# xiaozhah/Aligner

Hardware: AMD Instinct MI355X
Metric: aligned utterances/sec + frames/sec, [B=64,T_text=200,T_mel=1000] (higher is better)
Workload: dtype f32; 1 GPU; configs[1]: similarity (L2, C=80) + monotonic alignment search, [B=64,T_text=200,T_mel=1000] fp32 per GPU, dense fp32 path + int32 durations out; batch_per_gpu=64, t_text=200, t_mel=1000, c_att=80, launch=hipGraph, batches_in_flight=3, parallelism=batch-sharded x1

## Files before the change

aligner_amd/csrc/maxpath.hip:

```cpp
#include <hip/hip_runtime.h>

#include <climits>
#include <cstdint>
#include <cstring>
#include <type_traits>

#include "aligner_amd.h"
#include "common.h"
#include "device.h"
#include "maxpath_sweep_asm.inc"
#include "maxpath_walk_asm.inc"

namespace aligner {

constexpr int TC       = 32;
constexpr int TILE_LD  = 36;
constexpr int RING_T   = 4;
constexpr int RING_LD  = 64;
constexpr int RPW      = 63;
constexpr int WS_HDR_BYTES = 256;
constexpr int MV_CHUNKS = 32;

enum Mode { MODE_NORMAL = 0, MODE_EMPTY = 1, MODE_COMPAT = 2 };

typedef __attribute__((address_space(3))) float lds_float;
typedef float __attribute__((ext_vector_type(4))) f32x4;
typedef __attribute__((address_space(3))) f32x4 lds_f32x4;

struct MaxpathParams {
    const void  *value;
    const void  *mask;
    const int   *t_xs;
    const int   *t_ys;
    int         *starts;
    int         *tok;
    int         *dur;
    unsigned    *bits;
    int         *status;
    int         *mflag;
    int          verify;
    int          redo;
    int          ldv;
    int B, Tx, Ty, NT, ROWS;
    int WT;
    int bits_in_lds;
    int lds_bits_off;
    int lds_prev_off;
    int force_exact;
    float neg;
    int flags;
    float *qout;
    int lds_total;
    unsigned    *xring;
    int         *xflag;
    unsigned    *xwalk;
    int          split_walk;
    unsigned long long *stamps;
    float       *dump;
    void        *path1;
    int          path1_es;
    unsigned long long path1_one;
    int          zero_blocks;
    int          zero_nt;
    unsigned long long zero_n16;
    int         *zsync;
};

#define ALIGNER_STAMP(k)                                                                        \
    do {                                                                                        \
        if (p.stamps && (threadIdx.x & 63) == 0)                                                \
            p.stamps[((size_t)blockIdx.x * 16 + (threadIdx.x >> 6)) * 16 + (k)] =                \
                ((k) == 6 || (k) == 7) ? __builtin_amdgcn_s_memrealtime() : __builtin_amdgcn_s_memtime();   \
    } while (0)

constexpr int ZERO_SPIN_LIMIT = 1 << 22;

enum { VT_F32 = 0, VT_BF16 = 1, VT_F16 = 2 };

template <int VT> __device__ __forceinline__ float half_to_f32(unsigned h16) {
    if (VT == VT_BF16) return __builtin_bit_cast(float, h16 << 16);
    return (float)__builtin_bit_cast(_Float16, (unsigned short)h16);
}
template <int VT> __device__ __forceinline__ float mul_in_dtype(float v, float m) {
    const float r = v * m;
    if (VT == VT_BF16) return (float)(__bf16)r;
    if (VT == VT_F16) return (float)(_Float16)r;
    return r;
}
template <int VT> __device__ __forceinline__ float load_score(const void *base, size_t idx) {
    if (VT == VT_F32) return static_cast<const float *>(base)[idx];
    return half_to_f32<VT>(static_cast<const unsigned short *>(base)[idx]);
}
__device__ __forceinline__ float dpp_wave_shr1(float old_lane0, float src) {
    return __builtin_bit_cast(
        float, __builtin_amdgcn_update_dpp(__builtin_bit_cast(int, old_lane0),
                                           __builtin_bit_cast(int, src),
                                           0x138 , 0xf, 0xf, false));
}

__device__ __forceinline__ float comp(const float4 &v, int i) {
    return i == 0 ? v.x : i == 1 ? v.y : i == 2 ? v.z : v.w;
}

__device__ __forceinline__ int classify_lengths(const MaxpathParams &p, int b, int &tx, int &ty) {
    tx = p.t_xs[b];
    ty = p.t_ys[b];
    int st = 0;
    if (tx > p.Tx) { tx = p.Tx; st |= ALIGNER_ST_CLAMPED; }
    if (ty > p.Ty) { ty = p.Ty; st |= ALIGNER_ST_CLAMPED; }
    int mode;
    if (tx >= 1 && tx <= ty) {
        mode = MODE_NORMAL;
    } else if (ty <= 0) {
        mode = MODE_EMPTY;
        ty = 0;
        if (tx < 0) tx = 0;
    } else if (tx > ty && (p.flags & ALIGNER_F_COMPAT_TXGTTY)) {
        mode = MODE_COMPAT;
    } else {
        mode = MODE_EMPTY;
        st |= ALIGNER_ST_BAD_LENGTHS;
        if (tx < 0) tx = 0;
    }
    if (st && threadIdx.x == 0) atomicOr(p.status, st);
    return mode;
}

__device__ __forceinline__ bool tile_in_band(int t, int r0, int nrows, int tx, int ty) {
    const int y_lo = r0;
    const int y_hi = ty - tx + r0 + nrows - 1;
    return (TC * t + TC - 1 >= y_lo) && (TC * t <= y_hi);
}

__device__ __forceinline__ int starts_words_of(int Tx) { return ((Tx + 1 + 63) / 64) * 64 + 64; }

__device__ __forceinline__ void store_outputs(const MaxpathParams &p, int b, int tx, int ty, int *startsL,
                                              bool distinct_starts = true, int x_lo = 0, int x_hi = -1, int y_lo = 0,
                                              int y_hi = -1) {
    const int tid = threadIdx.x, nthreads = blockDim.x;
    if (p.path1 && p.zero_blocks > 0) {
        int gave_up = 0;
        if (tid == 0) {
            const int limit = (p.flags & ALIGNER_F_TEST_DROP_ZERO_REPORTS) ? (1 << 10) : ZERO_SPIN_LIMIT;
            int spins = 0;
            while (__hip_atomic_load(p.zsync, __ATOMIC_RELAXED, __HIP_MEMORY_SCOPE_AGENT) < p.zero_blocks) {
                if (++spins > limit) { atomicOr(p.status, ALIGNER_ST_INTERNAL); gave_up = 1; break; }
                __builtin_amdgcn_s_sleep(8);
            }
        }
        if (__syncthreads_or(gave_up)) {
            for (int x = tid; x <= p.Tx; x += nthreads) startsL[x] = 0;
            __syncthreads();
            tx = 0;
            ty = 0;
        }
    }
    const int xs_hi = x_hi < 0 ? p.Tx + 1 : x_hi, xd_hi = x_hi < 0 ? p.Tx : x_hi;
    const int ye = y_hi < 0 ? p.Ty : y_hi;
    for (int x = x_lo + tid; x < xs_hi; x += nthreads) p.starts[(size_t)b * (p.Tx + 1) + x] = startsL[x];
    if (p.dur)
        for (int x = x_lo + tid; x < xd_hi; x += nthreads) p.dur[(size_t)b * p.Tx + x] = startsL[x + 1] - startsL[x];
    if (!p.tok && !p.path1) return;
// ... 895 lines not shown
                walk_half(p, win2, RP2, ntb, x, e, 0, startsL + r0, lane);
                e = __builtin_amdgcn_readfirstlane(e);
                if (lane == 0) {
                    unsigned expect = XRING_EMPTY;
                    const bool ok = x == -1 && e >= r0 - 1 &&
                                    __hip_atomic_compare_exchange_strong(p.xwalk + b, &expect, (unsigned)e, __ATOMIC_RELAXED,
                                                                         __ATOMIC_RELAXED, __HIP_MEMORY_SCOPE_AGENT);
                    const bool cancelled = !ok && expect == XWALK_CANCEL;
                    if (!ok && !cancelled) {
                        if (expect == XRING_EMPTY)
                            __hip_atomic_store(p.xwalk + b, XWALK_SOLO, __ATOMIC_RELAXED, __HIP_MEMORY_SCOPE_AGENT);
                        atomicOr(p.status, ALIGNER_ST_INTERNAL);
                    }
                    *bcast = ok ? 1 : cancelled ? 2 : 0;
                }
            }
            ALIGNER_STAMP(3);
            __syncthreads();
            const int handed = *bcast;
            __syncthreads();
            if (handed == 0) {
                write_degenerate<MASKMODE, VT>(p, b, MODE_EMPTY, tx, ty, reinterpret_cast<int *>(smem));
                return;
            }
            if (handed == 1) {
                for (int r = tx + tid; r <= p.Tx; r += NW * 128) startsL[r] = ty;
                __syncthreads();
                store_outputs(p, b, tx, ty, startsL, true, r0, -1, startsL[r0], -1);
                ALIGNER_STAMP(5);
                ALIGNER_STAMP(7);
                return;
            }
            __threadfence_block();
            backtrack_and_store<(NW <= 4)>(p, b, tx, ty, smem);
            return;
        }
        if (p.split_walk && tid == 0) __hip_atomic_store(p.xwalk + b, XWALK_SOLO, __ATOMIC_RELAXED, __HIP_MEMORY_SCOPE_AGENT);
    }
    if (p.force_exact || flagp[0] != 0) exact_fallback_sweep<MASKMODE, VT>(p, b, tx, ty, smem, bitsL, RPB);
    __threadfence_block();
    ALIGNER_STAMP(1);
    backtrack_and_store<(NW <= 4)>(p, b, tx, ty, smem);
    ALIGNER_STAMP(5);
    ALIGNER_STAMP(7);
}

template <int VT, int NTHREADS>
__device__ __forceinline__ void verify_mask_piece(const MaxpathParams &p, int q) {
    constexpr int ES = VT == VT_F32 ? 4 : 2, EPV = 16 / ES, NWV = NTHREADS / 64;
    typedef typename std::conditional<ES == 4, unsigned, unsigned short>::type U;
    const unsigned one_bits = VT == VT_F32 ? 0x3F800000u : VT == VT_BF16 ? 0x3F80u : 0x3C00u;
    const unsigned w1 = ES == 4 ? one_bits : (one_bits | (one_bits << 16));
    const int b = q / MV_CHUNKS, c = q - b * MV_CHUNKS, tid = threadIdx.x, lane = tid & 63, wave = tid >> 6;
    const int tx = p.t_xs[b], ty = p.t_ys[b];
    int bad = 0;
    if (!(tx >= 1 && tx <= ty && tx <= p.Tx && ty <= p.Ty)) {
        bad = 1;
    } else {
        const U *mu = static_cast<const U *>(p.mask) + (size_t)b * p.Tx * p.Ty;
        const int per = (tx + MV_CHUNKS - 1) / MV_CHUNKS;
        const int r0 = c * per, r1 = r0 + per < tx ? r0 + per : tx;
        const bool vec = (p.Ty % EPV == 0) && ((reinterpret_cast<uintptr_t>(p.mask) & 15) == 0);
        const int nq = vec ? ty / EPV : 0;
        for (int x = r0 + wave; x < r1; x += NWV) {
            const uint4 *row = reinterpret_cast<const uint4 *>(mu + (size_t)x * p.Ty);
            int k = lane;
            for (; k + 192 < nq; k += 256) {
                const uint4 v0 = row[k], v1 = row[k + 64], v2 = row[k + 128], v3 = row[k + 192];
                bad |= (v0.x != w1) | (v0.y != w1) | (v0.z != w1) | (v0.w != w1) | (v1.x != w1) | (v1.y != w1) |
                       (v1.z != w1) | (v1.w != w1) | (v2.x != w1) | (v2.y != w1) | (v2.z != w1) | (v2.w != w1) |
                       (v3.x != w1) | (v3.y != w1) | (v3.z != w1) | (v3.w != w1);
            }
            for (; k < nq; k += 64) {
                const uint4 v = row[k];
                bad |= (v.x != w1) | (v.y != w1) | (v.z != w1) | (v.w != w1);
            }
            for (int y = nq * EPV + lane; y < ty; y += 64) bad |= mu[(size_t)x * p.Ty + y] != (U)one_bits;
        }
    }
    const int any = __syncthreads_or(bad);
    if (tid == 0) p.mflag[q] = any;
}

__device__ __forceinline__ void erase_path_ones(const MaxpathParams &p, int b) {
    const int *st = p.starts + (size_t)b * (p.Tx + 1);
    for (int x = threadIdx.x; x < p.Tx; x += blockDim.x) {
        const int s0 = st[x], s1 = st[x + 1];
        for (int y = s0; y < s1 && y < p.Ty; ++y) {
            const size_t idx = ((size_t)b * p.Tx + x) * p.Ty + y;
            switch (p.path1_es) {
                case 1: static_cast<unsigned char *>(p.path1)[idx] = 0; break;
                case 2: static_cast<unsigned short *>(p.path1)[idx] = 0; break;
                case 4: static_cast<unsigned *>(p.path1)[idx] = 0u; break;
                default: static_cast<unsigned long long *>(p.path1)[idx] = 0ull; break;
            }
        }
    }
    asm volatile("s_waitcnt vmcnt(0)" ::: "memory");
    __syncthreads();
}

template <int NW, int DEPTH, bool VEC, int MASKMODE, int VT, bool PAIR = false>
__global__ __launch_bounds__(NW * 128, 1) void maxpath_pipelined_kernel(MaxpathParams p) {
    const int Z = p.zero_blocks;
    if ((int)blockIdx.x < Z) {
        typedef unsigned u32x4 __attribute__((ext_vector_type(4)));
        u32x4 *d = reinterpret_cast<u32x4 *>(p.path1);
        const u32x4 z = {0u, 0u, 0u, 0u};
        const unsigned long long per = (p.zero_n16 + Z - 1) / Z;
        const unsigned long long lo = per * blockIdx.x, hi = lo + per < p.zero_n16 ? lo + per : p.zero_n16;
        if (p.zero_nt) {
            for (unsigned long long i = lo + threadIdx.x; i < hi; i += NW * 128)
                asm volatile("global_store_dwordx4 %0, %1, off sc1 nt" :: "v"(d + i), "v"(z) : "memory");
        } else {
            for (unsigned long long i = lo + threadIdx.x; i < hi; i += NW * 128)
                asm volatile("global_store_dwordx4 %0, %1, off sc1" :: "v"(d + i), "v"(z) : "memory");
        }
        asm volatile("s_waitcnt vmcnt(0)" ::: "memory");
        __syncthreads();
        if (threadIdx.x == 0 && !(p.flags & ALIGNER_F_TEST_DROP_ZERO_REPORTS))
            __hip_atomic_fetch_add(p.zsync, 1, __ATOMIC_RELAXED, __HIP_MEMORY_SCOPE_AGENT);
        if (MASKMODE == 0 && p.verify)
            for (int q = blockIdx.x; q < p.B * MV_CHUNKS; q += Z) verify_mask_piece<VT, NW * 128>(p, q);
    } else if (MASKMODE == 1 && p.redo) {
        const int b = (int)blockIdx.x;
        static_assert(MV_CHUNKS <= 64, "one flag word per lane");
        const int mine = (threadIdx.x & 63) < MV_CHUNKS ? p.mflag[b * MV_CHUNKS + (threadIdx.x & 63)] : 0;
        if (__builtin_amdgcn_ballot_w64(mine != 0) != 0) {
            if (p.path1) erase_path_ones(p, b);
            maxpath_pipelined_body<NW, DEPTH, VEC, 1, VT, PAIR>(p, b);
        }
    } else if (MASKMODE == 2) {
        const int blk = (int)blockIdx.x - Z;
        const int b = PAIR ? (blk >= p.B ? blk - p.B : blk) : blk;
        static_assert(MV_CHUNKS <= 64, "one flag word per lane");
        const int mine = (threadIdx.x & 63) < MV_CHUNKS ? p.mflag[b * MV_CHUNKS + (threadIdx.x & 63)] : 0;
        if (__builtin_amdgcn_ballot_w64(mine != 0) != 0) maxpath_pipelined_body<NW, DEPTH, VEC, 1, VT, PAIR>(p, blk);
        else maxpath_pipelined_body<NW, DEPTH, VEC, 0, VT, PAIR>(p, blk);
    } else {
        maxpath_pipelined_body<NW, DEPTH, VEC, MASKMODE, VT, PAIR>(p, (int)blockIdx.x - Z);
    }
    if (Z > 0) {
        __syncthreads();
        if (threadIdx.x == 0) {
            const int f = __hip_atomic_fetch_add(p.zsync + 1, 1, __ATOMIC_RELAXED, __HIP_MEMORY_SCOPE_AGENT);
            if (f == Z + (PAIR ? 2 : 1) * p.B - 1) {
                __hip_atomic_store(p.zsync, 0, __ATOMIC_RELAXED, __HIP_MEMORY_SCOPE_AGENT);
                __hip_atomic_store(p.zsync + 1, 0, __ATOMIC_RELAXED, __HIP_MEMORY_SCOPE_AGENT);
            }
        }
    }
}

template <typename T, bool VEC, bool STREAM>
__global__ __launch_bounds__(256) void expand_kernel(const int *__restrict__ starts, T *__restrict__ path,
                                                      int Tx, int Ty, int rows_per_block, T one) {
    const int b = blockIdx.z;
    const int x0 = blockIdx.y * rows_per_block;
    const int y0 = (blockIdx.x * 256 + threadIdx.x) * 4;
    if (y0 >= Ty) return;
    const int x1 = (x0 + rows_per_block < Tx) ? x0 + rows_per_block : Tx;
    const int *st = starts + (size_t)b * (Tx + 1);
    struct alignas(sizeof(T) * 4) Vec4 { T v[4]; };
    int s = st[x0];
    for (int x = x0; x < x1; ++x) {
        const int e = st[x + 1];
        T *dst = path + ((size_t)b * Tx + x) * Ty + y0;
        Vec4 o;
#pragma unroll
        for (int i = 0; i < 4; ++i) o.v[i] = (y0 + i >= s && y0 + i < e) ? one : T(0);
        if (VEC) {
            if (STREAM) {
                typedef T TV __attribute__((ext_vector_type(4)));
                TV ov;
                ov.x = o.v[0]; ov.y = o.v[1]; ov.z = o.v[2]; ov.w = o.v[3];
                __builtin_nontemporal_store(ov, reinterpret_cast<TV *>(dst));
            } else {
                *reinterpret_cast<Vec4 *>(dst) = o;
            }
        } else {
#pragma unroll
            for (int i = 0; i < 4; ++i)
                if (y0 + i < Ty) dst[i] = o.v[i];
        }
        s = e;
    }
}

template <typename T, int VT> __device__ __forceinline__ float mask_value(T v) {
    if (VT == VT_F32) return (float)v;
    return half_to_f32<VT>((unsigned)v);
}

template <typename T, int VT = VT_F32>
__global__ __launch_bounds__(256) void lengths_kernel(const T *__restrict__ mask, int Tx, int Ty,
                                                       int *__restrict__ t_xs, int *__restrict__ t_ys) {
    __shared__ float red[2][4];
    const int b = blockIdx.x, tid = threadIdx.x;
    const T *m = mask + (size_t)b * Tx * Ty;
    float sx = 0.f, sy = 0.f;
    for (int x = tid; x < Tx; x += 256) sx += mask_value<T, VT>(m[(size_t)x * Ty]);
    for (int y = tid; y < Ty; y += 256) sy += mask_value<T, VT>(m[y]);
#pragma unroll
    for (int off = 32; off > 0; off >>= 1) {
        sx += __shfl_down(sx, off);
        sy += __shfl_down(sy, off);
    }
    if ((tid & 63) == 0) { red[0][tid >> 6] = sx; red[1][tid >> 6] = sy; }
    __syncthreads();
    if (tid == 0) {
        t_xs[b] = (int)(red[0][0] + red[0][1] + red[0][2] + red[0][3]);
        t_ys[b] = (int)(red[1][0] + red[1][1] + red[1][2] + red[1][3]);
    }
}

template <int ES, int VT>
__global__ __launch_bounds__(256) void mask_verify_kernel(const void *__restrict__ maskv, int Tx, int Ty,
                                                           const int *__restrict__ t_xs_in, const int *__restrict__ t_ys_in,
                                                           int *__restrict__ t_xs_out, int *__restrict__ t_ys_out,
                                                           int *__restrict__ flag, unsigned one_bits) {
    __shared__ float red[2][4];
    __shared__ int anybad;
    typedef typename std::conditional<ES == 4, float, unsigned short>::type E;
    typedef typename std::conditional<ES == 4, unsigned, unsigned short>::type U;
    constexpr int EPV = 16 / ES;
    constexpr int NQ = 4;
    const int c = blockIdx.x, b = blockIdx.y, tid = threadIdx.x, lane = tid & 63, wave = tid >> 6;
    const E *m = static_cast<const E *>(maskv) + (size_t)b * Tx * Ty;
    const U *mu = reinterpret_cast<const U *>(m);
    const U one = (U)one_bits;
    const unsigned w1 = ES == 4 ? one_bits : (one_bits | (one_bits << 16));
    if (tid == 0) anybad = 0;
    const bool given = t_xs_in != nullptr;
    int tx = given ? t_xs_in[b] : -1, ty = given ? t_ys_in[b] : 0;
    const int rows = given ? (tx < Tx ? (tx > 0 ? tx : 0) : Tx) : Tx;
    const int per = (rows + MV_CHUNKS - 1) / MV_CHUNKS;
    const int r0 = c * per, r1 = r0 + per < rows ? r0 + per : rows;
    const bool vec = (Ty % EPV == 0) && ((reinterpret_cast<uintptr_t>(maskv) & 15) == 0);
    const int nqrow = Ty / EPV;
    auto fetch = [&](int x, uint4 (&v)[NQ], U &before) {
        const uint4 *row = reinterpret_cast<const uint4 *>(mu + (size_t)x * Ty);
#pragma unroll
        for (int i = 0; i < NQ; ++i) {
            const int q = lane + 64 * i;
            v[i] = row[q < nqrow ? q : nqrow - 1];
        }
        before = x > 0 ? mu[(size_t)(x - 1) * Ty] : one;
    };
    uint4 v[NQ];
    U before = one;
    int x = r0 + wave;
    if (vec && x < r1) fetch(x, v, before);
    if (!given) {
        float sx = 0.f, sy = 0.f;
        for (int y = tid; y < Ty; y += 256) sy += mask_value<E, VT>(m[y]);
        if (c == 0)
            for (int xx = tid; xx < Tx; xx += 256) sx += mask_value<E, VT>(m[(size_t)xx * Ty]);
#pragma unroll
        for (int off = 32; off > 0; off >>= 1) {
            sx += __shfl_down(sx, off);
            sy += __shfl_down(sy, off);
        }
        if (lane == 0) { red[0][wave] = sx; red[1][wave] = sy; }
    }
    __syncthreads();
    if (!given) {
        ty = (int)(red[1][0] + red[1][1] + red[1][2] + red[1][3]);
        if (c == 0) {
            tx = (int)(red[0][0] + red[0][1] + red[0][2] + red[0][3]);
            if (tid == 0) { t_xs_out[b] = tx; t_ys_out[b] = ty; }
        }
    }
    int bad = 0;
    if (tx >= 0 && !(tx >= 1 && tx <= ty && tx <= Tx && ty <= Ty)) bad = 1;
    if (ty < 1 || ty > Ty) bad = 1;
    if (!bad) {
        const int nq = vec ? ty / EPV : 0;
        for (; x < r1; x += 4) {
            bool inside = true;
            if (vec) {
                const unsigned f0 = __builtin_amdgcn_readfirstlane(v[0].x);
                const U first = (U)(ES == 4 ? f0 : (f0 & 0xFFFFu));
                if (!given) {
                    bad |= (first != one && first != 0) | (first == one && before != one);
                    inside = first == one;
                }
                if (inside) {
#pragma unroll
                    for (int i = 0; i < NQ; ++i)
                        if (lane + 64 * i < nq) bad |= (v[i].x != w1) | (v[i].y != w1) | (v[i].z != w1) | (v[i].w != w1);
                    const uint4 *row = reinterpret_cast<const uint4 *>(mu + (size_t)x * Ty);
                    for (int q = lane + 64 * NQ; q < nq; q += 64) {
                        const uint4 w = row[q];
                        bad |= (w.x != w1) | (w.y != w1) | (w.z != w1) | (w.w != w1);
                    }
                }
                if (x + 4 < r1) fetch(x + 4, v, before);
            } else if (!given) {
                const U first = mu[(size_t)x * Ty], bf = x > 0 ? mu[(size_t)(x - 1) * Ty] : one;
                bad |= (first != one && first != 0) | (first == one && bf != one);
                inside = first == one;
            }
            if (inside)
                for (int y = nq * EPV + lane; y < ty; y += 64) bad |= mu[(size_t)x * Ty + y] != one;
        }
    }
    if (bad) anybad = 1;
    __syncthreads();
    if (tid == 0) flag[b * MV_CHUNKS + c] = anybad;
}


struct WsLayout {
    size_t status_off, len_off, mflag_off, starts_off, bits_off, dump_off, xring_off, xring_bytes, total;
    int NT, ROWS;
};

static WsLayout ws_layout(int B, int Tx, int Ty) {
    WsLayout L;
    L.NT = (Ty + TC - 1) / TC;
    const int rows_pipe = (Tx + RPW - 1) / RPW * RPW + 1;
    const int rows_plain = (Tx + 255) / 256 * 256;
    L.ROWS = ((rows_pipe > rows_plain ? rows_pipe : rows_plain) + 63) / 64 * 64;
    L.status_off = 0;
    L.len_off = WS_HDR_BYTES;
    L.mflag_off = L.len_off + (size_t)2 * B * sizeof(int);
    L.starts_off = align_up(L.mflag_off + (size_t)B * MV_CHUNKS * sizeof(int), 256);
    L.bits_off = align_up(L.starts_off + (size_t)B * (Tx + 1) * sizeof(int), 256);
    L.dump_off = align_up(L.bits_off + (size_t)B * L.NT * L.ROWS * sizeof(unsigned), 256);
    L.xring_off = align_up(L.dump_off + (size_t)B * 4 * 64 * sizeof(float), 256);
    L.xring_bytes = align_up((size_t)B * L.NT * TC * sizeof(unsigned) + (size_t)2 * B * sizeof(int), 256);
    L.total = L.xring_off + L.xring_bytes;
    return L;
}

static int lds_limit() { return device_lds_limit(); }

static size_t starts_bytes(int Tx) { return (size_t)(((Tx + 1 + 63) / 64) * 64 + 64) * 4; }
// ... 149 lines not shown
    MaxpathParams p;
    p.value = value;
    p.mask = (flags & ALIGNER_F_STRICT_MASK) ? mask : nullptr;
    p.t_xs = t_xs; p.t_ys = t_ys;
    p.starts = reinterpret_cast<int *>(wsb + L.starts_off);
    p.tok = tok_out;
    p.dur = dur_out;
    p.bits = reinterpret_cast<unsigned *>(wsb + L.bits_off);
    p.status = reinterpret_cast<int *>(wsb + L.status_off);
    p.mflag = reinterpret_cast<int *>(wsb + L.mflag_off);
    p.verify = 0; p.redo = 0; p.ldv = ldv;
    p.B = B; p.Tx = Tx; p.Ty = Ty; p.NT = L.NT; p.ROWS = L.ROWS;
    p.neg = neg; p.flags = flags;
    p.bits_in_lds = 0; p.lds_bits_off = 0; p.lds_prev_off = 0;
    p.force_exact = !(neg - neg == 0.0f);
    p.stamps = g_debug_stamps;
    p.dump = nullptr;
    p.qout = nullptr;
    p.path1 = nullptr; p.path1_es = 0; p.path1_one = 0;
    if (path_prezeroed) set_path_ones(p, path_prezeroed, path_dtype);
    p.zero_blocks = 0; p.zero_nt = 0; p.zero_n16 = 0;
    p.zsync = reinterpret_cast<int *>(wsb + L.status_off + 16);
    if (path_prezeroed && path_done) *path_done = true;
    p.xring = reinterpret_cast<unsigned *>(wsb + L.xring_off);
    p.xflag = reinterpret_cast<int *>(wsb + L.xring_off + (size_t)B * L.NT * TC * sizeof(unsigned));
    p.xwalk = reinterpret_cast<unsigned *>(p.xflag + B);
    p.split_walk = 0;
    if (flags & ALIGNER_F_WRITE_Q) {
        if (vt != VT_F32 || (flags & ALIGNER_F_STRICT_MASK))
            return fail(ALIGNER_EINVAL, "ALIGNER_F_WRITE_Q takes fp32 scores without a strict mask (maximum_path_c's contract)");
        p.qout = const_cast<float *>(static_cast<const float *>(value));
        flags |= ALIGNER_F_FORCE_GENERIC;
        p.flags = flags;
    }
    const int maskmode = (flags & ALIGNER_F_STRICT_MASK) ? 1 : 0;
    const int pipemask = dyn_mask ? 2 : opt_mask ? 0 : maskmode;
    const size_t lds_max = (size_t)lds_limit();
    const int per16 = vt == VT_F32 ? 4 : 8;
    const bool vec = (Ty % per16 == 0) && (ldv % per16 == 0) && ((reinterpret_cast<uintptr_t>(value) & 15) == 0) &&
                     (!maskmode || (reinterpret_cast<uintptr_t>(mask) & 15) == 0) &&
                     (size_t)Tx * (size_t)ldv * 4 < (1ull << 31);

    const int nw_need = (Tx + RPW - 1) / RPW;
    if (!(flags & (ALIGNER_F_FORCE_GENERIC | ALIGNER_F_ONE_CU)) && nw_need > 4 && nw_need <= 8 && vec && ldv == Ty &&
        2 * B <= device_cu_count() &&
        ((flags & ALIGNER_F_TWO_CUS) || (8 * B <= device_cu_count() && L.NT >= 56))) {
        const size_t fwd = align_up(((size_t)4 * (2 * 64 * TILE_LD + RING_T * RING_LD) + RING_T * RING_LD) * 4 + 16, 16);
        p.WT = pick_window(L.NT, L.ROWS, Tx, lds_max);
        if (p.WT > 0 && fwd <= lds_max && starts_bytes(Tx) <= fwd) {
            size_t lds = walk_bytes(p.WT, L.ROWS, Tx);
            if (lds < fwd) lds = fwd;
            const size_t split_lds = starts_bytes(Tx) + (size_t)L.NT * row_pitch(256) * 4;
            if (split_lds <= lds_max && !g_opt_maxpath_no_split_walk) {
                p.split_walk = 1;
                if (lds < split_lds) lds = split_lds;
            }
            const int n16 = (int)(L.xring_bytes / 16);
            hipLaunchKernelGGL(xring_fill_kernel, dim3((n16 + 255) / 256), dim3(256), 0, s,
                               reinterpret_cast<uint4 *>(wsb + L.xring_off), n16);
            ALIGNER_HIP_CHECK(hipGetLastError());
            {
                const int cus = device_cu_count();
                const size_t pbytes = path_out ? (size_t)B * Tx * Ty * dtype_size(path_dtype) : 0;
                if (path_out && !path_is_zero && !(flags & ALIGNER_F_SEPARATE_EXPAND) && cus - 2 * B >= 32 &&
                    (reinterpret_cast<uintptr_t>(path_out) & 15) == 0 && pbytes % 16 == 0 && dtype_size(path_dtype) > 0) {
                    p.zero_blocks = cus - 2 * B < 48 ? cus - 2 * B : 48;
                    if (g_opt_maxpath_zero_blocks > 0 && g_opt_maxpath_zero_blocks <= cus - 2 * B) p.zero_blocks = g_opt_maxpath_zero_blocks;
                    p.zero_nt = (flags & ALIGNER_F_STREAM_PATH) ? 1 : 0;
                    p.zero_n16 = pbytes / 16;
                    set_path_ones(p, path_out, path_dtype);
                    if (path_done) *path_done = true;
                }
            }
            return launch_pair(p, pipemask, vt, lds, s);
        }
    }
    if (!(flags & ALIGNER_F_FORCE_GENERIC) && nw_need <= 8 && (vt == VT_F32 || vec)) {
        const int NW = (nw_need <= 4 && vt != VT_F32) ? 4 : nw_need <= 1 ? 1 : nw_need <= 2 ? 2 : nw_need <= 4 ? 4 : 8;
        const size_t fwd = align_up((size_t)NW * (2 * 64 * TILE_LD + RING_T * RING_LD) * 4 + 16, 16);
        if (fwd <= lds_max && starts_bytes(Tx) <= fwd) {
            size_t lds = 0;
            const size_t bits_lds = (size_t)L.NT * row_pitch(L.ROWS) * 4;
            if (L.NT <= 64 && fwd + bits_lds <= lds_max) {
                p.bits_in_lds = 1;
                p.lds_bits_off = (int)fwd;
                p.WT = L.NT;
                lds = fwd + bits_lds;
                const size_t prev_lds = bits_lds + (size_t)row_pitch(L.ROWS) * 4;
                if (NW <= 4 && L.NT < 64 && lds + prev_lds <= lds_max && !(flags & ALIGNER_F_NO_PREV_TABLE)) {
                    p.lds_prev_off = (int)lds;
                    lds += prev_lds;
                }
            } else {
                p.WT = pick_window(L.NT, L.ROWS, Tx, lds_max);
                if (p.WT > 0) {
                    lds = walk_bytes(p.WT, L.ROWS, Tx);
                    if (lds < fwd) lds = fwd;
                }
            }
            if (lds) {
                const int cus = device_cu_count();
                const size_t pbytes = path_out ? (size_t)B * Tx * Ty * dtype_size(path_dtype) : 0;
                if (path_out && !path_is_zero && !(flags & ALIGNER_F_SEPARATE_EXPAND) && cus - B >= 32 &&
                    (reinterpret_cast<uintptr_t>(path_out) & 15) == 0 && pbytes % 16 == 0 && dtype_size(path_dtype) > 0) {
                    p.zero_blocks = cus - B;
                    if (!opt_mask) {
                        const long long need = (long long)(pbytes / ((size_t)775 * (size_t)Ty)) + 1;
                        const int zc = need < 48 ? 48 : (int)(need > cus - B ? cus - B : need);
                        if (zc < p.zero_blocks) p.zero_blocks = zc;
                    }
                    if (g_opt_maxpath_zero_blocks >= 32 && g_opt_maxpath_zero_blocks <= cus - B) p.zero_blocks = g_opt_maxpath_zero_blocks;
                    p.zero_nt = (flags & ALIGNER_F_STREAM_PATH) ? 1 : 0;
                    p.zero_n16 = pbytes / 16;
                    set_path_ones(p, path_out, path_dtype);
                    if (path_done) *path_done = true;
                }
                auto launch = [&](const MaxpathParams &q, int mm) {
                    switch (NW) {
                        case 1: return launch_pipelined<1, 4>(q, vec, mm, vt, lds, s);
                        case 2: return launch_pipelined<2, 4>(q, vec, mm, vt, lds, s);
                        case 4: return launch_pipelined<4, 2>(q, vec, mm, vt, lds, s);
                        default: return launch_pipelined<8, 2>(q, vec, mm, vt, lds, s);
                    }
                };
                if (opt_mask && p.zero_blocks > 0) {
                    p.mask = mask;
                    p.verify = 1;
                    int rc = launch(p, 0);
                    if (rc != ALIGNER_OK) return rc;
                    MaxpathParams r = p;
                    r.verify = 0; r.redo = 1; r.zero_blocks = 0; r.zero_n16 = 0;
                    return launch(r, 1);
                }
                return launch(p, opt_mask ? maskmode : pipemask);
            }
        }
    }
    const int R = (Tx + 255) / 256;
    if (R > 8) return fail(ALIGNER_EDOM, "Tx=%d exceeds the 2048 text rows the kernels support", Tx);
    const int RR = R <= 1 ? 1 : R <= 2 ? 2 : R <= 4 ? 4 : 8;
    const size_t fwd = (size_t)2 * (256 * RR + 1) * 4;
    p.WT = pick_window(L.NT, L.ROWS, Tx, lds_max);
    if (p.WT <= 0) return fail(ALIGNER_EDOM, "Tx=%d/Ty=%d too large for the backtrack window", Tx, Ty);
    size_t lds = walk_bytes(p.WT, L.ROWS, Tx);
    if (lds < fwd) lds = fwd;
    switch (RR) {
        case 1: return launch_generic<1>(p, maskmode, vt, lds, s);
        case 2: return launch_generic<2>(p, maskmode, vt, lds, s);
        case 4: return launch_generic<4>(p, maskmode, vt, lds, s);
        default: return launch_generic<8>(p, maskmode, vt, lds, s);
    }
}

template <typename T>
static int launch_expand(const int *starts, void *path, int B, int Tx, int Ty, T one, bool stream_path, hipStream_t s) {
    int rpb = 8;
    if (stream_path) {
        const long long cells = (long long)B * ((Ty + 1023) / 1024) * Tx;
        const int want = (int)((cells + device_cu_count() - 1) / device_cu_count());
        rpb = want < 8 ? 8 : (want > Tx ? Tx : want);
    }
    dim3 grid((Ty + 1023) / 1024, (Tx + rpb - 1) / rpb, B), block(256);
    const bool vec = (Ty % 4 == 0) && ((reinterpret_cast<uintptr_t>(path) % (sizeof(T) * 4)) == 0);
    if (vec && stream_path)
        hipLaunchKernelGGL((expand_kernel<T, true, true>), grid, block, 0, s, starts, static_cast<T *>(path), Tx, Ty, rpb, one);
    else if (vec)
        hipLaunchKernelGGL((expand_kernel<T, true, false>), grid, block, 0, s, starts, static_cast<T *>(path), Tx, Ty, rpb, one);
    else
        hipLaunchKernelGGL((expand_kernel<T, false, false>), grid, block, 0, s, starts, static_cast<T *>(path), Tx, Ty, rpb, one);
    ALIGNER_HIP_CHECK(hipGetLastError());
    return ALIGNER_OK;
}

template <bool STREAM>
__global__ __launch_bounds__(256) void zero_path_kernel(uint4 *__restrict__ dst, size_t n16, unsigned char *__restrict__ tail,
                                                         int ntail) {
    const size_t stride = (size_t)gridDim.x * 256;
    typedef unsigned u32x4 __attribute__((ext_vector_type(4)));
    const u32x4 z = {0u, 0u, 0u, 0u};
    u32x4 *d = reinterpret_cast<u32x4 *>(dst);
    for (size_t i = (size_t)blockIdx.x * 256 + threadIdx.x; i < n16; i += stride) {
        if (STREAM) __builtin_nontemporal_store(z, d + i);
        else d[i] = z;
    }
    if (blockIdx.x == 0 && (int)threadIdx.x < ntail) tail[threadIdx.x] = 0;
}

template <typename T>
__global__ __launch_bounds__(256) void scatter_path_kernel(const int *__restrict__ starts, T *__restrict__ path, int Tx, int Ty,
                                                            T one) {
    extern __shared__ int st[];
    const int b = blockIdx.y, y = blockIdx.x * 256 + threadIdx.x;
    const int *sb = starts + (size_t)b * (Tx + 1);
    for (int x = threadIdx.x; x <= Tx; x += 256) st[x] = sb[x];
    __syncthreads();
    if (y >= Ty || y >= st[Tx] || y < st[0]) return;
    int lo = 0, hi = Tx;
    while (hi - lo > 1) {
        const int mid = (lo + hi) >> 1;
        if (st[mid] <= y) lo = mid;
        else hi = mid;
    }
    path[((size_t)b * Tx + lo) * Ty + y] = one;
}

template <typename T>
static int launch_scatter(const int *starts, void *path, int B, int Tx, int Ty, T one, hipStream_t s) {
    const size_t lds = (size_t)(Tx + 1) * sizeof(int);
    ALIGNER_HIP_CHECK(ensure_dynamic_lds(reinterpret_cast<const void *>(scatter_path_kernel<T>), lds));
    hipLaunchKernelGGL(scatter_path_kernel<T>, dim3((Ty + 255) / 256, B), dim3(256), lds, s, starts, static_cast<T *>(path),
                       Tx, Ty, one);
    ALIGNER_HIP_CHECK(hipGetLastError());
    return ALIGNER_OK;
}

static int expand_impl(const int *starts, void *path, int path_dtype, int B, int Tx, int Ty, bool stream_path, hipStream_t s) {
    if (B > 65535 || (Tx + 7) / 8 > 65535) return fail(ALIGNER_EDOM, "grid too large");
    switch (path_dtype) {
        case ALIGNER_DT_F32: return launch_expand<float>(starts, path, B, Tx, Ty, 1.0f, stream_path, s);
        case ALIGNER_DT_F64: return launch_expand<double>(starts, path, B, Tx, Ty, 1.0, stream_path, s);
        case ALIGNER_DT_I32: return launch_expand<int32_t>(starts, path, B, Tx, Ty, 1, stream_path, s);
        case ALIGNER_DT_I64: return launch_expand<int64_t>(starts, path, B, Tx, Ty, 1, stream_path, s);
        case ALIGNER_DT_U8:  return launch_expand<uint8_t>(starts, path, B, Tx, Ty, 1, stream_path, s);
        case ALIGNER_DT_F16: return launch_expand<uint16_t>(starts, path, B, Tx, Ty, 0x3C00, stream_path, s);
        case ALIGNER_DT_BF16: return launch_expand<uint16_t>(starts, path, B, Tx, Ty, 0x3F80, stream_path, s);
        default: return fail(ALIGNER_EINVAL, "path dtype %d not supported", path_dtype);
    }
}

}

using namespace aligner;

extern "C" {

size_t aligner_maxpath_workspace_bytes(int B, int Tx, int Ty) {
    if (B < 0 || Tx < 1 || Ty < 1) return 0;
    return ws_layout(B, Tx, Ty).total;
}

int aligner_lengths_from_mask(const void *mask, int mask_dtype, int B, int Tx, int Ty,
                              int32_t *t_xs, int32_t *t_ys, void *stream) {
    if (!mask || !t_xs || !t_ys) return fail(ALIGNER_EINVAL, "null pointer");
    if (B < 0 || Tx < 1 || Ty < 1) return fail(ALIGNER_EINVAL, "bad shape B=%d Tx=%d Ty=%d", B, Tx, Ty);
    if (B == 0) return ALIGNER_OK;
    hipStream_t s = static_cast<hipStream_t>(stream);
    switch (mask_dtype) {
        case ALIGNER_DT_F32:
            hipLaunchKernelGGL(lengths_kernel<float>, dim3(B), dim3(256), 0, s,
                               static_cast<const float *>(mask), Tx, Ty, t_xs, t_ys);
            break;
        case ALIGNER_DT_U8:
            hipLaunchKernelGGL(lengths_kernel<unsigned char>, dim3(B), dim3(256), 0, s,
                               static_cast<const unsigned char *>(mask), Tx, Ty, t_xs, t_ys);
            break;
        case ALIGNER_DT_I32:
            hipLaunchKernelGGL(lengths_kernel<int>, dim3(B), dim3(256), 0, s,
                               static_cast<const int *>(mask), Tx, Ty, t_xs, t_ys);
            break;
        case ALIGNER_DT_BF16:
            hipLaunchKernelGGL((lengths_kernel<unsigned short, VT_BF16>), dim3(B), dim3(256), 0, s,
                               static_cast<const unsigned short *>(mask), Tx, Ty, t_xs, t_ys);
            break;
        case ALIGNER_DT_F16:
            hipLaunchKernelGGL((lengths_kernel<unsigned short, VT_F16>), dim3(B), dim3(256), 0, s,
                               static_cast<const unsigned short *>(mask), Tx, Ty, t_xs, t_ys);
            break;
        default:
            return fail(ALIGNER_EINVAL, "mask dtype %d not supported (use F32, BF16, F16, U8 or I32)", mask_dtype);
    }
    ALIGNER_HIP_CHECK(hipGetLastError());
    return ALIGNER_OK;
}

int aligner_maxpath_forward(const void *value, int value_dtype, const void *mask, int mask_dtype,
                            const int32_t *t_xs, const int32_t *t_ys, int32_t *tok_out,
                            int32_t *dur_out, void *ws, size_t ws_bytes, int B, int Tx, int Ty,
                            float max_neg_val, int flags, void *stream) {
    return forward_impl(value, value_dtype, mask, mask_dtype, t_xs, t_ys, tok_out, dur_out, ws, ws_bytes, B, Tx, Ty,
                        max_neg_val, flags, static_cast<hipStream_t>(stream));
}

int aligner_maxpath_forward_f32(const float *value, const void *mask, int mask_dtype,
                                const int32_t *t_xs, const int32_t *t_ys, int32_t *tok_out,
                                int32_t *dur_out, void *ws, size_t ws_bytes, int B, int Tx, int Ty,
                                float max_neg_val, int flags, void *stream) {
    return forward_impl(value, ALIGNER_DT_F32, mask, mask_dtype, t_xs, t_ys, tok_out, dur_out, ws, ws_bytes, B, Tx, Ty,
                        max_neg_val, flags, static_cast<hipStream_t>(stream));
}

int aligner_maxpath_expand_ex(const void *ws, void *path, int path_dtype, int B, int Tx, int Ty, int flags,
                              void *stream) {
    if (!ws || !path) return fail(ALIGNER_EINVAL, "null pointer");
    if (B < 0 || Tx < 1 || Ty < 1) return fail(ALIGNER_EINVAL, "bad shape B=%d Tx=%d Ty=%d", B, Tx, Ty);
    if (B == 0) return ALIGNER_OK;
    const WsLayout L = ws_layout(B, Tx, Ty);
    const int *starts = reinterpret_cast<const int *>(static_cast<const unsigned char *>(ws) + L.starts_off);
    return expand_impl(starts, path, path_dtype, B, Tx, Ty, (flags & ALIGNER_F_STREAM_PATH) != 0,
                       static_cast<hipStream_t>(stream));
}

int aligner_maxpath_zero_path(void *path, int path_dtype, int B, int Tx, int Ty, int flags, void *stream) {
    if (!path) return fail(ALIGNER_EINVAL, "null pointer");
    if (B < 0 || Tx < 1 || Ty < 1) return fail(ALIGNER_EINVAL, "bad shape B=%d Tx=%d Ty=%d", B, Tx, Ty);
    const int es = dtype_size(path_dtype);
    if (es == 0) return fail(ALIGNER_EINVAL, "path dtype %d not supported", path_dtype);
    if (B == 0) return ALIGNER_OK;
    unsigned char *pb = static_cast<unsigned char *>(path);
    const size_t bytes = (size_t)B * Tx * Ty * es;
    hipStream_t s = static_cast<hipStream_t>(stream);
    const size_t head = (16 - (reinterpret_cast<uintptr_t>(pb) & 15)) & 15;
    const size_t h = head < bytes ? head : bytes;
    const size_t n16 = (bytes - h) / 16, tail = (bytes - h) - n16 * 16;
    if (h) {
        hipLaunchKernelGGL(zero_path_kernel<false>, dim3(1), dim3(256), 0, s, reinterpret_cast<uint4 *>(pb), (size_t)0, pb, (int)h);
        ALIGNER_HIP_CHECK(hipGetLastError());
    }
    size_t blocks = (n16 + 255) / 256;
    const size_t cap = (size_t)device_cu_count() * 16;
    blocks = blocks < 1 ? 1 : (blocks > cap ? cap : blocks);
    if (flags & ALIGNER_F_STREAM_PATH)
        hipLaunchKernelGGL(zero_path_kernel<true>, dim3((unsigned)blocks), dim3(256), 0, s, reinterpret_cast<uint4 *>(pb + h), n16,
                           pb + h + n16 * 16, (int)tail);
    else
        hipLaunchKernelGGL(zero_path_kernel<false>, dim3((unsigned)blocks), dim3(256), 0, s, reinterpret_cast<uint4 *>(pb + h), n16,
                           pb + h + n16 * 16, (int)tail);
    ALIGNER_HIP_CHECK(hipGetLastError());
    return ALIGNER_OK;
}

int aligner_maxpath_scatter_path(const void *ws, void *path, int path_dtype, int B, int Tx, int Ty, void *stream) {
    if (!ws || !path) return fail(ALIGNER_EINVAL, "null pointer");
    if (B < 0 || Tx < 1 || Ty < 1) return fail(ALIGNER_EINVAL, "bad shape B=%d Tx=%d Ty=%d", B, Tx, Ty);
    if (B == 0) return ALIGNER_OK;
    if (B > 65535) return fail(ALIGNER_EDOM, "grid too large");
    if ((size_t)(Tx + 1) * sizeof(int) > (size_t)device_lds_limit()) return fail(ALIGNER_EDOM, "Tx=%d too large", Tx);
    const WsLayout L = ws_layout(B, Tx, Ty);
    const int *starts = reinterpret_cast<const int *>(static_cast<const unsigned char *>(ws) + L.starts_off);
    hipStream_t s = static_cast<hipStream_t>(stream);
    switch (path_dtype) {
        case ALIGNER_DT_F32: return launch_scatter<float>(starts, path, B, Tx, Ty, 1.0f, s);
        case ALIGNER_DT_F64: return launch_scatter<double>(starts, path, B, Tx, Ty, 1.0, s);
        case ALIGNER_DT_I32: return launch_scatter<int32_t>(starts, path, B, Tx, Ty, 1, s);
        case ALIGNER_DT_I64: return launch_scatter<int64_t>(starts, path, B, Tx, Ty, 1, s);
        case ALIGNER_DT_U8:  return launch_scatter<uint8_t>(starts, path, B, Tx, Ty, 1, s);
        case ALIGNER_DT_F16: return launch_scatter<uint16_t>(starts, path, B, Tx, Ty, 0x3C00, s);
        case ALIGNER_DT_BF16: return launch_scatter<uint16_t>(starts, path, B, Tx, Ty, 0x3F80, s);
        default: return fail(ALIGNER_EINVAL, "path dtype %d not supported", path_dtype);
    }
}

int aligner_maxpath_expand(const void *ws, void *path, int path_dtype, int B, int Tx, int Ty,
                           void *stream) {
    return aligner_maxpath_expand_ex(ws, path, path_dtype, B, Tx, Ty, 0, stream);
}

int aligner_maxpath(const void *value, int value_dtype, const void *mask, int mask_dtype, const int32_t *t_xs,
                    const int32_t *t_ys, void *path_out, int path_dtype, int32_t *tok_out,
                    int32_t *dur_out, void *ws, size_t ws_bytes, int B, int Tx, int Ty,
                    float max_neg_val, int flags, void *stream) {
    if (path_out && dtype_size(path_dtype) == 0)
        return fail(ALIGNER_EINVAL, "path dtype %d not supported", path_dtype);
    const bool prez = path_out && (flags & ALIGNER_F_PATH_PREZEROED);
    bool path_done = false;
    int rc = forward_impl(value, value_dtype, mask, mask_dtype, t_xs, t_ys, tok_out, dur_out, ws, ws_bytes, B, Tx, Ty,
                          max_neg_val, flags, static_cast<hipStream_t>(stream), path_out, path_dtype, prez, &path_done);
    if (rc || !path_out || B == 0 || path_done) return rc;
    return aligner_maxpath_expand_ex(ws, path_out, path_dtype, B, Tx, Ty, flags, stream);
}

int aligner_maxpath_ld(const void *value, int value_dtype, int ld_value, const int32_t *t_xs, const int32_t *t_ys,
                       void *path_out, int path_dtype, int32_t *tok_out, int32_t *dur_out, void *ws, size_t ws_bytes, int B,
                       int Tx, int Ty, float max_neg_val, int flags, void *stream) {
    if (path_out && dtype_size(path_dtype) == 0)
        return fail(ALIGNER_EINVAL, "path dtype %d not supported", path_dtype);
// ... 72 lines not shown
```

Baseline: 2.148 million utterances/s.

## Rewrite path expansion as flat cache-line-aligned chunk stream with LDS-staged starts

Replaces the per-row 2D-grid expand kernel with a flat kernel that treats the whole B×Tx×Ty path tensor as a linear stream of 16-byte chunks. Chunks are aligned to 128-byte lines and walked in 256-chunk rounds, so each wavefront writes contiguous full lines, with work split evenly across CUs. Each workgroup stages the starts range it needs into LDS and uses magic-number division to find its (b,x,y) position, then advances incrementally. It also adds an element-wise fallback for unaligned shapes and drops the old grid-size limit. The cost is more index arithmetic per chunk and an LDS staging step.

```diff
diff --git a/aligner_amd/csrc/expand_lines.h b/aligner_amd/csrc/expand_lines.h
--- /dev/null
+++ b/aligner_amd/csrc/expand_lines.h
@@ -0,0 +1,109 @@
+#pragma once
+#include <stdint.h>
+
+#if defined(__HIPCC__) || defined(__CUDACC__)
+#define EL_HD __host__ __device__ __forceinline__
+#else
+#define EL_HD inline
+#endif
+
+namespace aligner {
+
+constexpr int EL_CHUNK = 16;
+constexpr int EL_LINE = 128;
+constexpr int EL_ROUND = 256;
+
+EL_HD bool el_chunked(uintptr_t base, int Ty, int es) {
+    return ((int64_t)Ty * es) % EL_CHUNK == 0 && base % EL_CHUNK == 0;
+}
+
+struct ExpandPlan {
+    int64_t first;
+    int64_t total;
+    int64_t span;
+    int wgs;
+};
+
+EL_HD ExpandPlan el_plan(uintptr_t base, int64_t elements, int es, int wgs_wanted) {
+    ExpandPlan g;
+    g.first = (int64_t)(base % EL_LINE) / EL_CHUNK;
+    g.total = g.first + elements * es / EL_CHUNK;
+    const int64_t rounds = (g.total + EL_ROUND - 1) / EL_ROUND;
+    int64_t wgs = wgs_wanted < 1 ? 1 : wgs_wanted;
+    if (wgs > rounds) wgs = rounds;
+    const int64_t per = (rounds + wgs - 1) / wgs;
+    g.span = per * EL_ROUND;
+    g.wgs = (int)((rounds + per - 1) / per);
+    return g;
+}
+
+EL_HD int64_t el_wg_begin(const ExpandPlan &g, int w) { return (int64_t)w * g.span; }
+EL_HD int64_t el_wg_end(const ExpandPlan &g, int w) {
+    const int64_t e = (int64_t)(w + 1) * g.span;
+    return e < g.total ? e : g.total;
+}
+template <typename I> EL_HD I el_lane_begin(const ExpandPlan &g, int w, int lane) {
+    const I c = (I)el_wg_begin(g, w) + (I)lane;
+    return c < (I)g.first ? c + EL_ROUND : c;
+}
+
+EL_HD bool el_fits32(const ExpandPlan &g, int epc) { return (g.total + EL_ROUND) * epc < ((int64_t)1 << 31); }
+
+template <typename I> struct ExpandDiv { I d; uint32_t m; int sh; };
+
+template <typename I> EL_HD ExpandDiv<I> el_div_by(int d) {
+    ExpandDiv<I> D;
+    D.d = (I)d;
+    int l = 0;
+    while (((int64_t)1 << l) < d) ++l;
+    D.sh = 31 + l;
+    D.m = (uint32_t)((((uint64_t)1 << D.sh) + (uint64_t)d - 1) / (uint64_t)d);
+    return D;
+}
+
+template <typename I> EL_HD I el_div(I n, const ExpandDiv<I> &D) {
+    if (sizeof(I) == 4) return (I)(((uint64_t)n * D.m) >> D.sh);
+    return n / D.d;
+}
+
+template <typename I>
+EL_HD void el_table_range(const ExpandPlan &g, int w, int epc, const ExpandDiv<I> &Tx, const ExpandDiv<I> &Ty, I &i0, I &count) {
+    const I b = (I)el_wg_begin(g, w), f = (I)g.first, c0 = b > f ? b : f;
+    const I r0 = el_div((c0 - f) * (I)epc, Ty), r1 = el_div(((I)el_wg_end(g, w) - f) * (I)epc - 1, Ty);
+    i0 = r0 + el_div(r0, Tx);
+    count = r1 + el_div(r1, Tx) + 2 - i0;
+}
+
+struct ExpandPos { int b, x, y; };
+
+template <typename I> EL_HD ExpandPos el_locate(I e, const ExpandDiv<I> &Tx, const ExpandDiv<I> &Ty) {
+    const I r = el_div(e, Ty), b = el_div(r, Tx);
+    ExpandPos p;
+    p.y = (int)(e - r * Ty.d);
+    p.x = (int)(r - b * Tx.d);
+    p.b = (int)b;
+    return p;
+}
+
+struct ExpandStep { int db, dx, dy; };
+
+EL_HD ExpandStep el_step(int64_t adv_elements, int Tx, int Ty) {
+    ExpandStep s;
+    const int64_t r = adv_elements / Ty;
+    s.dy = (int)(adv_elements - r * Ty);
+    s.db = (int)(r / Tx);
+    s.dx = (int)(r - (int64_t)s.db * Tx);
+    return s;
+}
+
+EL_HD void el_advance(ExpandPos &p, const ExpandStep &s, int Tx, int Ty) {
+    p.y += s.dy;
+    p.x += s.dx;
+    p.b += s.db;
+    if (p.y >= Ty) { p.y -= Ty; p.x += 1; }
+    if (p.x >= Tx) { p.x -= Tx; p.b += 1; }
+}
+
+EL_HD bool el_is_one(int s, int e, int y) { return y >= s && y < e; }
+
+}
diff --git a/aligner_amd/csrc/maxpath.hip b/aligner_amd/csrc/maxpath.hip
--- a/aligner_amd/csrc/maxpath.hip
+++ b/aligner_amd/csrc/maxpath.hip
@@ -8,6 +8,7 @@
 #include "aligner_amd.h"
 #include "common.h"
 #include "device.h"
+#include "expand_lines.h"
 #include "maxpath_sweep_asm.inc"
 #include "maxpath_walk_asm.inc"
 
@@ -1209,38 +1210,56 @@
     }
 }
 
-template <typename T, bool VEC, bool STREAM>
-__global__ __launch_bounds__(256) void expand_kernel(const int *__restrict__ starts, T *__restrict__ path,
-                                                      int Tx, int Ty, int rows_per_block, T one) {
-    const int b = blockIdx.z;
-    const int x0 = blockIdx.y * rows_per_block;
-    const int y0 = (blockIdx.x * 256 + threadIdx.x) * 4;
-    if (y0 >= Ty) return;
-    const int x1 = (x0 + rows_per_block < Tx) ? x0 + rows_per_block : Tx;
-    const int *st = starts + (size_t)b * (Tx + 1);
-    struct alignas(sizeof(T) * 4) Vec4 { T v[4]; };
-    int s = st[x0];
-    for (int x = x0; x < x1; ++x) {
-        const int e = st[x + 1];
-        T *dst = path + ((size_t)b * Tx + x) * Ty + y0;
-        Vec4 o;
+constexpr int EL_STAGE = 2048;
+template <typename U, typename I, bool STREAM, bool STAGED>
+__device__ __forceinline__ void expand_rounds(const int *__restrict__ tab, I i0, unsigned char *__restrict__ line0, I c, I end,
+                                              ExpandPos p, int Tx, int Ty, const ExpandStep &step, U one) {
+    constexpr int EPC = EL_CHUNK / (int)sizeof(U);
+    typedef unsigned u32x4 __attribute__((ext_vector_type(4)));
+    for (; c < end; c += EL_ROUND) {
+        const I at = (I)p.b * (I)(Tx + 1) + (I)p.x - i0;
+        const int s = tab[at], e = tab[at + 1];
+        union { U v[EPC]; u32x4 q; } o;
 #pragma unroll
-        for (int i = 0; i < 4; ++i) o.v[i] = (y0 + i >= s && y0 + i < e) ? one : T(0);
-        if (VEC) {
-            if (STREAM) {
-                typedef T TV __attribute__((ext_vector_type(4)));
-                TV ov;
-                ov.x = o.v[0]; ov.y = o.v[1]; ov.z = o.v[2]; ov.w = o.v[3];
-                __builtin_nontemporal_store(ov, reinterpret_cast<TV *>(dst));
-            } else {
-                *reinterpret_cast<Vec4 *>(dst) = o;
-            }
-        } else {
-#pragma unroll
-            for (int i = 0; i < 4; ++i)
-                if (y0 + i < Ty) dst[i] = o.v[i];
-        }
-        s = e;
+        for (int i = 0; i < EPC; ++i) o.v[i] = el_is_one(s, e, p.y + i) ? one : U(0);
+        u32x4 *dst = reinterpret_cast<u32x4 *>(line0 + (size_t)c * EL_CHUNK);
+        if (STREAM) __builtin_nontemporal_store(o.q, dst);
+        else *dst = o.q;
+        el_advance(p, step, Tx, Ty);
+    }
+}
+
+template <typename U, typename I, bool STREAM>
+__global__ __launch_bounds__(256) void expand_kernel(const int *__restrict__ starts, unsigned char *__restrict__ line0,
+                                                      ExpandDiv<I> dTx, ExpandDiv<I> dTy, ExpandPlan g, ExpandStep step, U one) {
+    constexpr int EPC = EL_CHUNK / (int)sizeof(U);
+    __shared__ int stL[EL_STAGE];
+    const int Tx = (int)dTx.d, Ty = (int)dTy.d;
+    const I end = (I)el_wg_end(g, blockIdx.x);
+    I i0, count;
+    el_table_range<I>(g, blockIdx.x, EPC, dTx, dTy, i0, count);
+    const bool staged = count <= (I)EL_STAGE;
+    if (staged)
+        for (unsigned i = threadIdx.x; i < (unsigned)count; i += 256) stL[i] = starts[i0 + i];
+    const I c = el_lane_begin<I>(g, blockIdx.x, threadIdx.x);
+    const ExpandPos p = el_locate<I>((c - (I)g.first) * EPC, dTx, dTy);
+    if (staged) {
+        __syncthreads();
+        expand_rounds<U, I, STREAM, true>(stL, i0, line0, c, end, p, Tx, Ty, step, one);
+    } else {
+        expand_rounds<U, I, STREAM, false>(starts, (I)0, line0, c, end, p, Tx, Ty, step, one);
+    }
+}
+
+template <typename U>
+__global__ __launch_bounds__(256) void expand_elements_kernel(const int *__restrict__ starts, U *__restrict__ path,
+                                                               int Tx, int Ty, size_t n, U one) {
+    const size_t stride = (size_t)gridDim.x * 256;
+    const ExpandDiv<uint64_t> dTx = el_div_by<uint64_t>(Tx), dTy = el_div_by<uint64_t>(Ty);
+    for (size_t i = (size_t)blockIdx.x * 256 + threadIdx.x; i < n; i += stride) {
+        const ExpandPos p = el_locate<uint64_t>(i, dTx, dTy);
+        const int *st = starts + (size_t)p.b * (Tx + 1) + p.x;
+        path[i] = el_is_one(st[0], st[1], p.y) ? one : U(0);
     }
 }
 
@@ -1696,22 +1715,33 @@
     }
 }
 
-template <typename T>
-static int launch_expand(const int *starts, void *path, int B, int Tx, int Ty, T one, bool stream_path, hipStream_t s) {
-    int rpb = 8;
-    if (stream_path) {
-        const long long cells = (long long)B * ((Ty + 1023) / 1024) * Tx;
-        const int want = (int)((cells + device_cu_count() - 1) / device_cu_count());
-        rpb = want < 8 ? 8 : (want > Tx ? Tx : want);
-    }
-    dim3 grid((Ty + 1023) / 1024, (Tx + rpb - 1) / rpb, B), block(256);
-    const bool vec = (Ty % 4 == 0) && ((reinterpret_cast<uintptr_t>(path) % (sizeof(T) * 4)) == 0);
-    if (vec && stream_path)
-        hipLaunchKernelGGL((expand_kernel<T, true, true>), grid, block, 0, s, starts, static_cast<T *>(path), Tx, Ty, rpb, one);
-    else if (vec)
-        hipLaunchKernelGGL((expand_kernel<T, true, false>), grid, block, 0, s, starts, static_cast<T *>(path), Tx, Ty, rpb, one);
-    else
-        hipLaunchKernelGGL((expand_kernel<T, false, false>), grid, block, 0, s, starts, static_cast<T *>(path), Tx, Ty, rpb, one);
+template <typename U>
+static int launch_expand(const int *starts, void *path, int B, int Tx, int Ty, U one, bool stream_path, hipStream_t s) {
+    const uintptr_t base = reinterpret_cast<uintptr_t>(path);
+    const long long n = (long long)B * Tx * Ty;
+    const int cus = device_cu_count();
+    if (!el_chunked(base, Ty, (int)sizeof(U))) {
+        long long blocks = (n + 255) / 256;
+        if (blocks > (long long)cus * 16) blocks = (long long)cus * 16;
+        hipLaunchKernelGGL(expand_elements_kernel<U>, dim3((unsigned)blocks), dim3(256), 0, s, starts, static_cast<U *>(path), Tx,
+                           Ty, (size_t)n, one);
+        ALIGNER_HIP_CHECK(hipGetLastError());
+        return ALIGNER_OK;
+    }
+    const ExpandPlan g = el_plan(base, n, (int)sizeof(U), stream_path ? cus : cus * 8);
+    const ExpandStep step = el_step(EL_ROUND * (EL_CHUNK / (long long)sizeof(U)), Tx, Ty);
+    unsigned char *line0 = reinterpret_cast<unsigned char *>(base - base % EL_LINE);
+    const dim3 grid((unsigned)g.wgs), block(256);
+#define EL_LAUNCH(I, STREAM)                                                                                          \
+    hipLaunchKernelGGL((expand_kernel<U, I, STREAM>), grid, block, 0, s, starts, line0, el_div_by<I>(Tx), el_div_by<I>(Ty), g, step, one)
+    if (el_fits32(g, EL_CHUNK / (int)sizeof(U))) {
+        if (stream_path) EL_LAUNCH(uint32_t, true);
+        else EL_LAUNCH(uint32_t, false);
+    } else {
+        if (stream_path) EL_LAUNCH(uint64_t, true);
+        else EL_LAUNCH(uint64_t, false);
+    }
+#undef EL_LAUNCH
     ALIGNER_HIP_CHECK(hipGetLastError());
     return ALIGNER_OK;
 }
@@ -1759,12 +1789,11 @@
 }
 
 static int expand_impl(const int *starts, void *path, int path_dtype, int B, int Tx, int Ty, bool stream_path, hipStream_t s) {
-    if (B > 65535 || (Tx + 7) / 8 > 65535) return fail(ALIGNER_EDOM, "grid too large");
     switch (path_dtype) {
-        case ALIGNER_DT_F32: return launch_expand<float>(starts, path, B, Tx, Ty, 1.0f, stream_path, s);
-        case ALIGNER_DT_F64: return launch_expand<double>(starts, path, B, Tx, Ty, 1.0, stream_path, s);
-        case ALIGNER_DT_I32: return launch_expand<int32_t>(starts, path, B, Tx, Ty, 1, stream_path, s);
-        case ALIGNER_DT_I64: return launch_expand<int64_t>(starts, path, B, Tx, Ty, 1, stream_path, s);
+        case ALIGNER_DT_F32: return launch_expand<uint32_t>(starts, path, B, Tx, Ty, 0x3F800000u, stream_path, s);
+        case ALIGNER_DT_F64: return launch_expand<uint64_t>(starts, path, B, Tx, Ty, 0x3FF0000000000000ull, stream_path, s);
+        case ALIGNER_DT_I32: return launch_expand<uint32_t>(starts, path, B, Tx, Ty, 1u, stream_path, s);
+        case ALIGNER_DT_I64: return launch_expand<uint64_t>(starts, path, B, Tx, Ty, 1ull, stream_path, s);
         case ALIGNER_DT_U8:  return launch_expand<uint8_t>(starts, path, B, Tx, Ty, 1, stream_path, s);
         case ALIGNER_DT_F16: return launch_expand<uint16_t>(starts, path, B, Tx, Ty, 0x3C00, stream_path, s);
         case ALIGNER_DT_BF16: return launch_expand<uint16_t>(starts, path, B, Tx, Ty, 0x3F80, stream_path, s);
```

Result: faster. 2.216 million utterances/s (median of 6 runs) (+3.1%).
